# FrozenBurning/SceneDreamer

Measured on AMD Instinct MI355X. Metric: rendered frames/sec @960×540, 24 samples/ray, scene_size 2048; HBM GB/s, higher is better.
Workload: dtype f16 (3-term split MFMA, f32 accumulate; f32 hash grid); 1 GPU; 960x540, num_samples=24, scene_size=2048, cam pattern 0 (pose stride 2 of 40 poses), 1 frame per rank per step; apron=minimal, parallelism=frames x1

## Files before the change

scenedreamer_amd/cnn.py:

```python
import ctypes
import os

import torch

from . import capi

_LAYERS = {"conv1": (64, 1), "conv2a": (256, 9), "conv2b": (256, 9), "conv3a": (256, 9), "conv3b": (256, 9),
           "conv4a": (256, 1), "conv4b": (256, 1)}
_3X3 = ("conv2a", "conv2b", "conv3a", "conv3b")
CNN_LADDER = (1, "1113", "1133", 3)


def form_key(terms3x3):
    if isinstance(terms3x3, (tuple, list)):
        terms3x3 = "".join(str(int(t)) for t in terms3x3)
    if isinstance(terms3x3, str):
        terms3x3 = terms3x3.strip()
        if terms3x3 in ("1", "3"):
            return int(terms3x3)
        if not (len(terms3x3) == 4 and set(terms3x3) <= {"1", "3"}):
            raise ValueError(f"3x3 precision form {terms3x3!r}: expected 1, 3 or four characters of 1 / 3 (conv2a, conv2b, conv3a, conv3b), e.g. 1113")
        return 1 if terms3x3 == "1111" else 3 if terms3x3 == "3333" else terms3x3
    assert int(terms3x3) in (1, 3), terms3x3
    return int(terms3x3)


def form_terms(terms3x3):
    k = form_key(terms3x3)
    return (k,) * 4 if isinstance(k, int) else tuple(int(c) for c in k)


def form_cost(terms3x3):
    return sum(form_terms(terms3x3))


class MfmaCNN:
    def __init__(self, R, terms3x3, chain=None):
        self.R = R
        self.form = form_key(terms3x3)
        per3x3 = dict(zip(_3X3, form_terms(terms3x3)))
        if chain is None:
            chain = os.environ.get("SDN_CNN_CHAIN", "1") != "0"
        self.chain = bool(chain)
        self.terms = {n: per3x3.get(n, 3) for n in _LAYERS}
        lib = capi.lib()
        w = R.w
        self.packed = {}
        with torch.cuda.device(R.dev):
            for n, (cin, taps) in _LAYERS.items():
                wt = w[f"denoiser.{n}.weight"]
                assert tuple(wt.shape[:2]) == (256, cin) and wt.shape[2] * wt.shape[3] == taps, (n, tuple(wt.shape))
                buf = torch.empty(lib.sdn_conv_packed_weight_bytes(cin, taps, self.terms[n]), dtype=torch.uint8, device=R.dev)
                capi.check(lib.sdn_conv_pack_weights(wt.contiguous().data_ptr(), cin, taps, self.terms[n], buf.data_ptr(),
                                                     capi.current_stream(R.dev)), "sdn_conv_pack_weights")
                self.packed[n] = buf
        self.w4 = w["denoiser.conv4.weight"].reshape(3, 256).contiguous()
        self.b4 = w["denoiser.conv4.bias"].contiguous()
        self._planes = {}
        if self.chain:
            from . import fused
            try:
                fused.check_trunk_range(w["denoiser.conv4a.weight"], [w["denoiser.conv4b.weight"], w["denoiser.conv4.weight"]],
                                        lib.sdn_field_trunk_shift(), "render CNN tail")
            except fused.TrunkRangeError as e:
                import warnings
                warnings.warn(f"MfmaCNN: {e}; head and tail run as sdn_conv launches instead (no pre-tanh output)")
                self.chain = False
        if self.chain:
            with torch.cuda.device(R.dev):
                self.chain_packed = torch.empty(lib.sdn_conv_chain_packed_weight_bytes(), dtype=torch.uint8, device=R.dev)
                w4a = w["denoiser.conv4a.weight"].reshape(256, 256).contiguous()
                w4b = w["denoiser.conv4b.weight"].reshape(256, 256).contiguous()
                capi.check(lib.sdn_conv_chain_pack_weights(w4a.data_ptr(), w4b.data_ptr(), self.w4.data_ptr(),
                                                           self.chain_packed.data_ptr(), capi.current_stream(R.dev)),
                           "sdn_conv_chain_pack_weights")
                c = torch.zeros(lib.sdn_conv_chain_consts_floats(), device=R.dev)
                c[0:256] = w["denoiser.conv4a.bias"]
                c[256:512] = w["denoiser.conv4b.bias"]
                c[512:515] = self.b4
                self.chain_consts = c
                self.head_packed = torch.empty(lib.sdn_conv_head_packed_weight_bytes(), dtype=torch.uint8, device=R.dev)
                w1 = w["denoiser.conv1.weight"].reshape(256, 64).contiguous()
                capi.check(lib.sdn_conv_head_pack_weights(w1.data_ptr(), self.head_packed.data_ptr(), capi.current_stream(R.dev)),
                           "sdn_conv_head_pack_weights")
                self.head_bias = w["denoiser.conv1.bias"].contiguous()

    def _buffers(self, H, W):
        key = (H, W)
        if key not in self._planes:
            hb, wb = ctypes.c_int(), ctypes.c_int()
            capi.lib().sdn_conv_plane_dims(H, W, ctypes.byref(hb), ctypes.byref(wb))
            n = hb.value * wb.value * 256
            mk = lambda: torch.zeros(n, dtype=torch.float16, device=self.R.dev)
            while len(self._planes) >= 2:
                self._planes.pop(next(iter(self._planes)))
            self._planes[key] = dict(a=(mk(), mk()), b=(mk(), mk()))
        return self._planes[key]

    def _adapt(self):
        t = self.R.cnn_adapt
        if getattr(self, "_adapt_src", None) is not t:
            self._adapt_src = t
            self._adapt_vecs = [c[0].contiguous() for c in torch.chunk(t, 4, dim=-1)]
        return self._adapt_vecs

    def _conv(self, src, name, H, W, bias=None, resid=None, resid_planes=None, mod=None, dst=None, out32=None, proj=None,
              img=None):
        p = lambda t: t.data_ptr() if t is not None else None
        cin, taps = _LAYERS[name]
        with torch.cuda.device(self.R.dev):
            capi.check(capi.lib().sdn_conv(src[0].data_ptr(), src[1].data_ptr(), cin, taps, self.terms[name],
                                           self.packed[name].data_ptr(),
                                           p(bias), p(resid), resid_planes[0].data_ptr() if resid_planes else None,
                                           resid_planes[1].data_ptr() if resid_planes else None,
                                           p(mod[0]) if mod else None, p(mod[1]) if mod else None,
                                           dst[0].data_ptr() if dst else None,
                                           dst[1].data_ptr() if dst and dst[1] is not None else None, p(out32),
                                           p(proj[0]) if proj else None, p(proj[1]) if proj else None, p(img),
                                           H, W, 0, capi.current_stream(self.R.dev)), "sdn_conv")

    FLOP_PER_PIXEL = {"head (conv1)": 2 * 64 * 256, "conv2a": 2 * 9 * 256 * 256, "conv2b": 2 * 9 * 256 * 256, "conv3a": 2 * 9 * 256 * 256,
                      "conv3b": 2 * 9 * 256 * 256, "chain (conv4a, conv4b, conv4)": 2 * (2 * 256 * 256 + 256 * 3)}

    def __call__(self, net_out, raw=None, timers=None):
        last = [None]

        def tick(name=None):
            if timers is None:
                return
            e = torch.cuda.Event(enable_timing=True)
            e.record()
            if name is not None:
                timers.setdefault(name, []).append((last[0], e))
            last[0] = e
        if raw is not None and not self.chain:
            raise ValueError("the pre-tanh output is produced by the chained tail (chain=True)")
        R, w = self.R, self.R.w
        _, H, W, _ = net_out.shape
        buf = self._buffers(H, W)
        A, B = buf["a"], buf["b"]
        a = self._adapt()
        bias = lambda n: w.get(f"denoiser.{n}.bias")
        x = net_out.reshape(H * W, 64).contiguous()
        img = torch.empty(1, 3, H, W, device=R.dev)
        tick()
        if self.chain:
            with torch.cuda.device(R.dev):
                capi.check(capi.lib().sdn_conv_head(x.data_ptr(), self.head_packed.data_ptr(), self.head_bias.data_ptr(),
                                                    A[0].data_ptr(), A[1].data_ptr(), H, W, 0, capi.current_stream(R.dev)),
                           "sdn_conv_head")
        else:
            with torch.cuda.device(R.dev):
                capi.check(capi.lib().sdn_conv_planes_from_f32(x.data_ptr(), 64, B[0].data_ptr(), B[1].data_ptr(), H, W,
                                                               capi.current_stream(R.dev)), "sdn_conv_planes_from_f32")
            self._conv(B, "conv1", H, W, bias=bias("conv1"), dst=A)
        inner = lambda consumer: (B[0], None) if self.terms[consumer] == 1 else B
        tick("head (conv1)")
        self._conv(A, "conv2a", H, W, bias=bias("conv2a"), dst=inner("conv2b"))
        tick("conv2a")
        self._conv(B, "conv2b", H, W, bias=bias("conv2b"), resid_planes=A, mod=(a[0], a[1]), dst=A)
        tick("conv2b")
        self._conv(A, "conv3a", H, W, bias=bias("conv3a"), dst=inner("conv3b"))
        tick("conv3a")
        self._conv(B, "conv3b", H, W, bias=bias("conv3b"), resid_planes=A, mod=(a[2], a[3]), dst=A)
        tick("conv3b")
        if self.chain:
            with torch.cuda.device(R.dev):
                capi.check(capi.lib().sdn_conv_chain(A[0].data_ptr(), A[1].data_ptr(), self.chain_packed.data_ptr(),
                                                     self.chain_consts.data_ptr(), img.data_ptr(),
                                                     raw.data_ptr() if raw is not None else None, H, W, 0,
                                                     capi.current_stream(R.dev)), "sdn_conv_chain")
            tick("chain (conv4a, conv4b, conv4)")
            return img
        self._conv(A, "conv4a", H, W, bias=bias("conv4a"), dst=B)
        self._conv(B, "conv4b", H, W, bias=bias("conv4b"), resid_planes=A, proj=(self.w4, self.b4), img=img)
        return img


class F32CNN:

    FLOP_PER_PIXEL = {"conv1": 2 * 64 * 256, "conv2a": 2 * 9 * 256 * 256, "conv2b": 2 * 9 * 256 * 256, "conv3a": 2 * 9 * 256 * 256,
                      "conv3b": 2 * 9 * 256 * 256, "conv4a": 2 * 256 * 256, "conv4b (+ conv4)": 2 * (256 * 256 + 256 * 3)}

    def __init__(self, R):
        self.R = R
        self._planes = {}
        lib = capi.lib()
        w = R.w
        self.packed = {}
        with torch.cuda.device(R.dev):
            for n, (cin, taps) in _LAYERS.items():
                wt = w[f"denoiser.{n}.weight"]
                assert tuple(wt.shape[:2]) == (256, cin) and wt.shape[2] * wt.shape[3] == taps, (n, tuple(wt.shape))
                buf = torch.empty(lib.sdn_conv_f32_packed_weight_bytes(cin, taps), dtype=torch.uint8, device=R.dev)
                capi.check(lib.sdn_conv_pack_weights_f32(wt.contiguous().data_ptr(), cin, taps, buf.data_ptr(), capi.current_stream(R.dev)),
                           "sdn_conv_pack_weights_f32")
                self.packed[n] = buf
        self.bias = {n: (w[f"denoiser.{n}.bias"].contiguous() if f"denoiser.{n}.bias" in w else None) for n in _LAYERS}
        self.w4 = w["denoiser.conv4.weight"].reshape(3, 256).contiguous()
        self.b4 = w["denoiser.conv4.bias"].contiguous()

    def _buffers(self, H, W):
# ... 55 lines not shown
```

scenedreamer_amd/csrc/cnn.hip:

```cpp
#include <hip/hip_fp16.h>

#include <cstdlib>

#include "mfma_common.h"
#include "sdn_common.h"

namespace {

typedef _Float16 half4 __attribute__((ext_vector_type(4)));

constexpr int CH = 256;
constexpr int A_BYTES = 16384;
constexpr int B_BYTES = 2048;
constexpr int WAVES = 8;
constexpr int SLOT_BYTES = A_BYTES + WAVES * B_BYTES;
constexpr int NSLOT = 5;
constexpr int AHEAD = 4;
constexpr int DMA_PER_SLOT = 4;
constexpr int TILE_W = 8, TILE_H = 4;
constexpr int PATCH_W = 16, PATCH_H = 16;

struct ConvParams {
    const _Float16 *xh, *xl;
    const char *wpk;
    int ksteps;
    const float *bias;
    const float *resid;
    const _Float16 *rh, *rl;
    const float *mod_w;
    const float *mod_b;
    _Float16 *oh, *ol;
    float *of32;
    const float *proj_w;
    const float *proj_b;
    float *img;
    int H, W, Hb, Wb;
    long chunk_bytes;
    unsigned row_inc, chunk_inc;
    int gx, gy, n_groups;
};

struct Stream {
    unsigned long off;
    int tap;
    int w;
};

template <int TAPS>
__device__ __forceinline__ void stream_advance_k(const ConvParams &p, Stream &st) {
    if constexpr (TAPS == 9) {
        unsigned inc = ((0x24u >> st.tap) & 1u) ? p.row_inc : 32u;
        inc = st.tap == 8 ? p.chunk_inc : inc;
        st.off += inc;
        st.tap = st.tap == 8 ? 0 : st.tap + 1;
    } else {
        st.off += (unsigned long)p.chunk_bytes;
    }
}

struct SlotIssue {
    const char *w;
    const char *a0, *a1;
    unsigned voff;
    char *dst;
};

template <int TAPS, int TERMS>
__device__ __forceinline__ SlotIssue stream_next_slot(const ConvParams &p, Stream &st, char *lds, int pos, int wave, unsigned voff, int ksteps) {
    SlotIssue si;
    si.w = p.wpk + (size_t)st.w * A_BYTES + wave * 2048;
    si.a0 = (const char *)p.xh + st.off;
    if constexpr (TERMS == 1) {
        stream_advance_k<TAPS>(p, st);
        si.a1 = (const char *)p.xh + st.off;
    } else {
        si.a1 = (const char *)p.xl + st.off;
    }
    stream_advance_k<TAPS>(p, st);
    st.w++;
    if (st.w == ksteps) {
        st.w = 0;
        st.off = 0;
    }
    si.voff = voff;
    si.dst = lds + pos * SLOT_BYTES;
    return si;
}

template <int TAPS, int TERMS, int U>
__device__ __forceinline__ void stream_chunk(const ConvParams &p, Stream &st, SlotIssue &sn, char *lds, int &pos, int wave,
                                             unsigned voff_sel, int ksteps) {
    if constexpr (U == 0) {
        asm volatile("" : "+s"(st.w));
        sn.w = p.wpk + (size_t)st.w * A_BYTES + wave * 2048;
        sn.dst = lds + pos * SLOT_BYTES;
        pos = pos + 1 == NSLOT ? 0 : pos + 1;
        asm volatile("" ::"s"(sn.w), "s"(pos));
    } else if constexpr (U == 1) {
        asm volatile("" : "+s"(st.tap));
        sn.a0 = (const char *)p.xh + st.off;
        if constexpr (TERMS == 1) stream_advance_k<TAPS>(p, st);
        asm volatile("" ::"s"(sn.a0), "s"(st.off), "s"(st.tap));
    } else if constexpr (U == 2) {
        asm volatile("" : "+s"(st.tap));
        sn.a1 = (const char *)(TERMS == 1 ? p.xh : p.xl) + st.off;
        stream_advance_k<TAPS>(p, st);
        asm volatile("" ::"s"(sn.a1), "s"(st.off), "s"(st.tap));
    } else {
        asm volatile("" : "+s"(st.w));
        st.w++;
        if (st.w == ksteps) {
            st.w = 0;
            st.off = 0;
        }
        asm volatile("" ::"s"(st.w), "s"(st.off));
    }
}

template <int PIECE>
__device__ __forceinline__ void issue_piece(const SlotIssue &si, int wave, int lane) {
    if constexpr (PIECE == 0) __builtin_amdgcn_global_load_lds((glb_char *)(si.w + (unsigned)(lane * 16)), (lds_char *)(si.dst + wave * 2048), 16, 0, 0);
    if constexpr (PIECE == 1) __builtin_amdgcn_global_load_lds((glb_char *)(si.w + (unsigned)(lane * 16)), (lds_char *)(si.dst + wave * 2048), 16, 1024, 0);
    if constexpr (PIECE == 2) __builtin_amdgcn_global_load_lds((glb_char *)(si.a0 + si.voff), (lds_char *)(si.dst + A_BYTES + wave * B_BYTES), 16, 0, 0);
    if constexpr (PIECE == 3) __builtin_amdgcn_global_load_lds((glb_char *)(si.a1 + si.voff), (lds_char *)(si.dst + A_BYTES + wave * B_BYTES + 1024), 16, 0, 0);
}

template <int TAPS, int TERMS, int DBG, int U>
__device__ __forceinline__ void conv_unit(f32x16 (&acc)[8], half8 (&a)[4][4], half8 (&bcur)[2], half8 (&bnext)[2], unsigned slot,
                                          unsigned slot_n, unsigned b_off, const SlotIssue &si, int wave, int lane,
                                          const ConvParams &p, Stream &st, SlotIssue &sn, char *lds, int &pos_issue, unsigned voff_sel, int ksteps) {
    constexpr int ib = 2 * U;
    half8(&au)[4] = a[U];
    half8(&nx)[4] = a[(U + 2) & 3];
    const unsigned src = U < 2 ? slot : slot_n;
    constexpr int OFF = ((U + 2) & 3) * 4096;
    if constexpr (!(DBG & 64)) lds_wait<U == 3 ? 6 : 4>();
#define SDN_GAP(K) \
    if constexpr (K == 0 && !(DBG & 1)) issue_piece<U>(si, wave, lane); \
    if constexpr (K == 0 && U == 2 && !(DBG & 64)) { ds_read16<0>(bnext[0], slot_n + b_off); ds_read16<1024>(bnext[1], slot_n + b_off); } \
    if constexpr (K >= 1 && K <= 4 && !(DBG & 64)) ds_read16<OFF + (K - 1) * 1024>(nx[K - 1], src); \
    if constexpr (K == 2) stream_chunk<TAPS, TERMS, U>(p, st, sn, lds, pos_issue, wave, voff_sel, ksteps); \
    __builtin_amdgcn_sched_barrier(0);
    if constexpr (DBG & 16) {
        asm volatile("" ::"v"(au[0]), "v"(au[1]), "v"(au[2]), "v"(au[3]), "v"(bcur[0]), "v"(bcur[1]));
        SDN_GAP(0) SDN_GAP(1) SDN_GAP(2) SDN_GAP(3) SDN_GAP(4)
    } else if constexpr (TERMS == 1) {
        acc[ib] = mfma16(au[0], bcur[0], acc[ib]);
        __builtin_amdgcn_sched_barrier(0);
        SDN_GAP(0)
        acc[ib + 1] = mfma16(au[2], bcur[0], acc[ib + 1]);
        SDN_GAP(1) SDN_GAP(2)
        acc[ib] = mfma16(au[1], bcur[1], acc[ib]);
        SDN_GAP(3)
        acc[ib + 1] = mfma16(au[3], bcur[1], acc[ib + 1]);
        SDN_GAP(4)
    } else {
        acc[ib] = mfma16(au[0], bcur[0], acc[ib]);
        __builtin_amdgcn_sched_barrier(0);
        SDN_GAP(0)
        acc[ib + 1] = mfma16(au[2], bcur[0], acc[ib + 1]);
        SDN_GAP(1)
        acc[ib] = mfma16(au[1], bcur[0], acc[ib]);
        SDN_GAP(2)
        acc[ib + 1] = mfma16(au[3], bcur[0], acc[ib + 1]);
        SDN_GAP(3)
        acc[ib] = mfma16(au[0], bcur[1], acc[ib]);
        SDN_GAP(4)
        acc[ib + 1] = mfma16(au[2], bcur[1], acc[ib + 1]);
        __builtin_amdgcn_sched_barrier(0);
    }
#undef SDN_GAP
}

__device__ __forceinline__ long lane_pixel_offset(const ConvParams &p, int grp, int wave, int lane, int &py, int &px) {
    const int gyi = grp / p.gx, gxi = grp - gyi * p.gx;
    const int j = lane & 31, h = lane >> 5;
    py = gyi * PATCH_H + (wave >> 1) * TILE_H + (j >> 3);
    px = gxi * PATCH_W + (wave & 1) * TILE_W + (j & 7);
    return ((long)(py + 1) * p.Wb + (px + 1)) * 32 + h * 16;
}

template <int TAPS, int DBG, int TERMS, int EPI>
__global__ __launch_bounds__(512, 2) void conv_kernel(const ConvParams p) {
    __shared__ __attribute__((aligned(1024))) char lds[NSLOT * SLOT_BYTES];
    const int lane = threadIdx.x & 63;
    const int wave = __builtin_amdgcn_readfirstlane(threadIdx.x >> 6);
    const int h = lane >> 5;

    int grp = blockIdx.x;
    if (grp >= p.n_groups) return;
    const unsigned tap0 = TAPS == 9 ? (unsigned)(p.Wb + 1) * 32u : 0u;
    int py, px;
    unsigned voff = (unsigned)lane_pixel_offset(p, grp, wave, lane, py, px) - tap0;
    int grp_n = grp + gridDim.x;
    int pyn, pxn;
    unsigned voff_n = grp_n < p.n_groups ? (unsigned)lane_pixel_offset(p, grp_n, wave, lane, pyn, pxn) - tap0 : voff;

    const int ksteps = p.ksteps;
    {
        const int n_mine = (p.n_groups - (int)blockIdx.x + (int)gridDim.x - 1) / (int)gridDim.x;
        const int n_max = (p.n_groups + (int)gridDim.x - 1) / (int)gridDim.x;
        if (!(DBG & 2048) && n_mine < n_max) {
            const int phase = (blockIdx.x >> 3) & 15;
            const int naps = (phase * (ksteps * 1400 + 20000)) >> (4 + 13);
            for (int i = 0; i < naps; i++) __builtin_amdgcn_s_sleep(127);
        }
    }
    Stream st{0ul, 0, 0};
    int pos_issue = 0, pos_use = 0;
#pragma unroll
    for (int q = 0; q < AHEAD; q++) {
        const SlotIssue si = stream_next_slot<TAPS, TERMS>(p, st, lds, pos_issue, wave, voff, ksteps);
        issue_piece<0>(si, wave, lane);
        issue_piece<1>(si, wave, lane);
        issue_piece<2>(si, wave, lane);
        issue_piece<3>(si, wave, lane);
        pos_issue = pos_issue + 1 == NSLOT ? 0 : pos_issue + 1;
    }
    SlotIssue si = stream_next_slot<TAPS, TERMS>(p, st, lds, pos_issue, wave, AHEAD < ksteps ? voff : voff_n, ksteps);
    pos_issue = pos_issue + 1 == NSLOT ? 0 : pos_issue + 1;

    half8 a[4][4];
    half8 b[2][2];
    const unsigned lds_lane = lds_addr(lds) + lane * 16;
    const unsigned b_off = A_BYTES + wave * B_BYTES;
    bool first_patch = true;
    asm volatile("s_waitcnt vmcnt(%0)" ::"n"((AHEAD - 1) * DMA_PER_SLOT) : "memory");
    __builtin_amdgcn_s_barrier();
    ds_read16<0>(b[0][0], lds_lane + b_off);
    ds_read16<1024>(b[0][1], lds_lane + b_off);
    lds_unit<0>(lds_lane, a[0]);
    lds_unit<1>(lds_lane, a[1]);

    while (true) {
        f32x16 acc[8];
#pragma unroll
        for (int ib = 0; ib < 8; ib++)
#pragma unroll
            for (int r = 0; r < 16; r++) acc[ib][r] = 0.f;
#pragma unroll 1
        for (int kt2 = 0; kt2 < ksteps; kt2 += 2) {
#pragma unroll
            for (int par = 0; par < 2; par++) {
                const int kt = kt2 + par;
                SlotIssue sn;
                si.voff = kt + AHEAD < ksteps ? voff : voff_n;
                const unsigned voff_sel = si.voff;
                const unsigned slot = lds_lane + pos_use * SLOT_BYTES;
                pos_use = pos_use + 1 == NSLOT ? 0 : pos_use + 1;
                const unsigned slot_n = lds_lane + pos_use * SLOT_BYTES;
                asm volatile("" ::"v"(voff_sel), "v"(slot), "v"(slot_n));
                __builtin_amdgcn_sched_barrier(0);
                if (kt >= AHEAD - 1 || first_patch) asm volatile("s_waitcnt vmcnt(%0)" ::"n"((AHEAD - 2) * DMA_PER_SLOT) : "memory");
                if constexpr (!(DBG & 2)) __builtin_amdgcn_s_barrier();
                __builtin_amdgcn_sched_barrier(0);
                conv_unit<TAPS, TERMS, DBG, 0>(acc, a, b[par], b[par ^ 1], slot, slot_n, b_off, si, wave, lane, p, st, sn, lds, pos_issue, voff_sel, ksteps);
                conv_unit<TAPS, TERMS, DBG, 1>(acc, a, b[par], b[par ^ 1], slot, slot_n, b_off, si, wave, lane, p, st, sn, lds, pos_issue, voff_sel, ksteps);
                conv_unit<TAPS, TERMS, DBG, 2>(acc, a, b[par], b[par ^ 1], slot, slot_n, b_off, si, wave, lane, p, st, sn, lds, pos_issue, voff_sel, ksteps);
                conv_unit<TAPS, TERMS, DBG, 3>(acc, a, b[par], b[par ^ 1], slot, slot_n, b_off, si, wave, lane, p, st, sn, lds, pos_issue, voff_sel, ksteps);
                si = sn;
            }
        }
        asm volatile("s_waitcnt vmcnt(0) lgkmcnt(0)" ::: "memory");
        first_patch = false;

        const bool in_frame = py < p.H && px < p.W;
        if (in_frame) {
            const long orow = (long)py * p.W + px;
            const long ppix = (long)(py + 1) * p.Wb + (px + 1);
            float pj[3] = {0.f, 0.f, 0.f};
            const long plane_px = (long)p.Hb * p.Wb;
            constexpr bool SPEC = EPI != 255;
            const bool has_bias = SPEC ? !(EPI & 8) : p.bias != nullptr, has_rp = SPEC ? bool(EPI & 1) : p.rh != nullptr;
            const bool has_mod = SPEC ? bool(EPI & 2) : p.mod_w != nullptr, has_r32 = !SPEC && p.resid;
            const bool has_proj = !SPEC && p.proj_w, has_o32 = !SPEC && p.of32;
            const bool has_oh = SPEC || p.oh, has_ol = SPEC ? bool(EPI & 16) : p.ol != nullptr;
            int he = h;
            asm volatile("" : "+v"(he));
#pragma unroll
            for (int ib = 0; ib < 8; ib++) {
#pragma unroll
                for (int q = 0; q < 2; q++) {
                    const int c0 = 32 * ib + 16 * he + 8 * q;
                    const long po = ((long)(2 * ib + he) * plane_px + ppix) * 16 + 8 * q;
                    float v[8];
#pragma unroll
                    for (int e = 0; e < 8; e++) v[e] = acc[ib][8 * q + e];
                    if (has_bias) {
                        const float4 b0 = *reinterpret_cast<const float4 *>(p.bias + c0), b1 = *reinterpret_cast<const float4 *>(p.bias + c0 + 4);
                        v[0] += b0.x; v[1] += b0.y; v[2] += b0.z; v[3] += b0.w; v[4] += b1.x; v[5] += b1.y; v[6] += b1.z; v[7] += b1.w;
                    }
                    if (has_r32) {
                        const float4 r0 = *reinterpret_cast<const float4 *>(p.resid + orow * CH + c0);
                        const float4 r1 = *reinterpret_cast<const float4 *>(p.resid + orow * CH + c0 + 4);
                        v[0] = r0.x + v[0]; v[1] = r0.y + v[1]; v[2] = r0.z + v[2]; v[3] = r0.w + v[3];
                        v[4] = r1.x + v[4]; v[5] = r1.y + v[5]; v[6] = r1.z + v[6]; v[7] = r1.w + v[7];
                    } else if (has_rp) {
                        const half8 h8 = *reinterpret_cast<const half8 *>(p.rh + po);
                        const half8 l8 = *reinterpret_cast<const half8 *>(p.rl + po);
#pragma unroll
                        for (int e = 0; e < 8; e++) v[e] = ((float)h8[e] + (float)l8[e]) + v[e];
                    }
                    if (has_mod) {
#pragma unroll
                        for (int e4 = 0; e4 < 2; e4++) {
                            const float4 mw = *reinterpret_cast<const float4 *>(p.mod_w + c0 + 4 * e4);
                            const float4 mb = *reinterpret_cast<const float4 *>(p.mod_b + c0 + 4 * e4);
                            v[4 * e4] = v[4 * e4] * (mw.x + 1.f) + mb.x; v[4 * e4 + 1] = v[4 * e4 + 1] * (mw.y + 1.f) + mb.y;
                            v[4 * e4 + 2] = v[4 * e4 + 2] * (mw.z + 1.f) + mb.z; v[4 * e4 + 3] = v[4 * e4 + 3] * (mw.w + 1.f) + mb.w;
                        }
                    }
#pragma unroll
                    for (int e = 0; e < 8; e++) v[e] = vmax(v[e], 0.2f * v[e]);
                    if (has_proj) {
#pragma unroll
                        for (int c = 0; c < 3; c++) {
                            const float4 w0 = *reinterpret_cast<const float4 *>(p.proj_w + c * CH + c0);
                            const float4 w1 = *reinterpret_cast<const float4 *>(p.proj_w + c * CH + c0 + 4);
                            pj[c] += w0.x * v[0] + w0.y * v[1] + w0.z * v[2] + w0.w * v[3] + w1.x * v[4] + w1.y * v[5] + w1.z * v[6] + w1.w * v[7];
                        }
                    }
#pragma unroll
                    for (int e = 0; e < 8; e++) acc[ib][8 * q + e] = v[e];
                }
            }
            if (has_o32 || has_oh) {
#pragma unroll
                for (int ib = 0; ib < 8; ib++) {
#pragma unroll
                    for (int q = 0; q < 2; q++) {
                        const int c0 = 32 * ib + 16 * he + 8 * q;
                        const long po = ((long)(2 * ib + he) * plane_px + ppix) * 16 + 8 * q;
                        float v[8];
#pragma unroll
                        for (int e = 0; e < 8; e++) v[e] = acc[ib][8 * q + e];
                        if (has_o32) {
                            *reinterpret_cast<float4 *>(p.of32 + orow * CH + c0) = make_float4(v[0], v[1], v[2], v[3]);
                            *reinterpret_cast<float4 *>(p.of32 + orow * CH + c0 + 4) = make_float4(v[4], v[5], v[6], v[7]);
                        }
                        if (has_oh) {
                            half8 hv, lv;
#pragma unroll
                            for (int e = 0; e < 8; e += 2) {
                                const half2v hp = cvt_rtn(v[e], v[e + 1]);
                                hv[e] = hp[0]; hv[e + 1] = hp[1];
                                const half2v lp = cvt_rtn(v[e] - (float)hp[0], v[e + 1] - (float)hp[1]);
                                lv[e] = lp[0]; lv[e + 1] = lp[1];
                            }
                            *reinterpret_cast<half8 *>(p.oh + po) = hv;
                            if (has_ol) *reinterpret_cast<half8 *>(p.ol + po) = lv;
                        }
                    }
                }
            }
            if (has_proj) {
#pragma unroll
                for (int c = 0; c < 3; c++) {
                    const float t = pj[c] + __shfl_xor(pj[c], 32);
                    if (h == 0) p.img[(long)c * p.H * p.W + orow] = tanhf(t + p.proj_b[c]);
                }
            }
        }
        grp = grp_n;
        if (grp >= p.n_groups) break;
        voff = voff_n;
        py = pyn;
        px = pxn;
        grp_n = grp + gridDim.x;
        voff_n = grp_n < p.n_groups ? (unsigned)lane_pixel_offset(p, grp_n, wave, lane, pyn, pxn) - tap0 : voff;
    }
    asm volatile("s_waitcnt vmcnt(0)" ::: "memory");
    __builtin_amdgcn_s_barrier();
}

__global__ __launch_bounds__(256) void pack_conv_kernel(const float *__restrict__ W, half8 *__restrict__ out, int cin, int taps, int terms) {
    const size_t g = (size_t)blockIdx.x * 256 + threadIdx.x;
    const int nslots = (cin / 16) * taps / (terms == 1 ? 2 : 1);
    if (g >= (size_t)nslots * 8 * 64) return;
    const int lane = (int)(g % 64);
    const int ib = (int)((g / 64) % 8);
    const int t = (int)(g / (64 * 8));
    const int i32 = lane & 31, h = lane >> 5;
    const int co = 32 * ib + 16 * ((i32 >> 2) & 1) + 4 * (i32 >> 3) + (i32 & 3);
    half8 hi, lo;
    if (terms == 1) {
#pragma unroll
        for (int kk = 0; kk < 2; kk++) {
            const int k = 2 * t + kk, s = k / taps, tap = k - taps * s;
#pragma unroll
            for (int e = 0; e < 8; e++) {
                const _Float16 vh = (_Float16)W[((size_t)co * cin + 16 * s + 8 * h + e) * taps + tap];
                if (kk == 0) hi[e] = vh;
                else lo[e] = vh;
            }
        }
    } else {
        const int s = t / taps, tap = t - taps * s;
#pragma unroll
        for (int e = 0; e < 8; e++) {
            const int ci = 16 * s + 8 * h + e;
            const float v = W[((size_t)co * cin + ci) * taps + tap];
            const _Float16 vh = (_Float16)v;
            hi[e] = vh;
            lo[e] = (_Float16)(v - (float)vh);
        }
    }
    const size_t base = ((size_t)t * 16 + (size_t)(ib / 2) * 4 + (ib & 1) * 2) * 64 + lane;
    out[base] = hi;
    out[base + 64] = lo;
}

__global__ __launch_bounds__(256) void planes_kernel(const float *__restrict__ x, _Float16 *__restrict__ oh,
                                                     _Float16 *__restrict__ ol, int H, int W, int Hb, int Wb, int C) {
    const long n = (long)H * W * (C / 4);
    for (long i = (long)blockIdx.x * 256 + threadIdx.x; i < n; i += (long)gridDim.x * 256) {
        const long pix = i / (C / 4);
        const int c0 = (int)(i % (C / 4)) * 4;
        const int y = (int)(pix / W), xx = (int)(pix % W);
        const float4 v = *reinterpret_cast<const float4 *>(x + pix * C + c0);
        const half2v h0 = cvt_rtn(v.x, v.y), h1 = cvt_rtn(v.z, v.w);
        const half2v l0 = cvt_rtn(v.x - (float)h0[0], v.y - (float)h0[1]);
        const half2v l1 = cvt_rtn(v.z - (float)h1[0], v.w - (float)h1[1]);
        half4 hv, lv;
        hv[0] = h0[0]; hv[1] = h0[1]; hv[2] = h1[0]; hv[3] = h1[1];
        lv[0] = l0[0]; lv[1] = l0[1]; lv[2] = l1[0]; lv[3] = l1[1];
        const long o = ((long)(c0 >> 4) * ((long)Hb * Wb) + (long)(y + 1) * Wb + (xx + 1)) * 16 + (c0 & 15);
        *reinterpret_cast<half4 *>(oh + o) = hv;
        *reinterpret_cast<half4 *>(ol + o) = lv;
    }
}

}

extern "C" {

void sdn_conv_plane_dims(int H, int W, int *Hb, int *Wb) {
    *Hb = sdn::div_up(H, PATCH_H) * PATCH_H + 2;
    *Wb = sdn::div_up(W, PATCH_W) * PATCH_W + 2;
}

static bool conv_shape_ok(int cin, int taps, int terms) {
    if (terms != 1 && terms != 3) return false;
    if (terms == 1 && !(taps == 9 && cin == 256)) return false;
    return (taps == 9 && cin == 256) || (taps == 1 && cin >= 64 && cin <= 256 && cin % 16 == 0);
}
#define SDN_CONV_SHAPES "supported: 3x3 256->256 (terms 1 or 3) and 1x1 (64..256, multiple of 16)->256 (terms 3)"

static int conv_slots(int cin, int taps, int terms) { return (cin / 16) * taps / (terms == 1 ? 2 : 1); }

size_t sdn_conv_packed_weight_bytes(int cin, int taps, int terms) {
    return conv_shape_ok(cin, taps, terms) ? (size_t)conv_slots(cin, taps, terms) * A_BYTES : 0;
}

int sdn_conv_pack_weights(const float *w_oihw, int cin, int taps, int terms, void *packed, sdn_stream_t stream) {
    SDN_REQUIRE(w_oihw && packed, "sdn_conv_pack_weights: null pointer");
    SDN_REQUIRE(conv_shape_ok(cin, taps, terms), "sdn_conv_pack_weights: " SDN_CONV_SHAPES);
    const size_t n = (size_t)conv_slots(cin, taps, terms) * 8 * 64;
    hipLaunchKernelGGL(pack_conv_kernel, dim3((unsigned)sdn::div_up<size_t>(n, 256)), dim3(256), 0, (hipStream_t)stream,
                       w_oihw, (half8 *)packed, cin, taps, terms);
    return sdn::check_launch("sdn_conv_pack_weights");
}

int sdn_conv_planes_from_f32(const float *x, int channels, void *out_hi, void *out_lo, int H, int W, sdn_stream_t stream) {
    SDN_REQUIRE(x && out_hi && out_lo && H > 0 && W > 0, "sdn_conv_planes_from_f32: bad argument");
    SDN_REQUIRE(channels >= 16 && channels <= 256 && channels % 16 == 0, "sdn_conv_planes_from_f32: channels must be a multiple of 16 in [16, 256]");
    int Hb, Wb;
    sdn_conv_plane_dims(H, W, &Hb, &Wb);
    hipLaunchKernelGGL(planes_kernel, dim3(2048), dim3(256), 0, (hipStream_t)stream, x, (_Float16 *)out_hi, (_Float16 *)out_lo,
                       H, W, Hb, Wb, channels);
    return sdn::check_launch("sdn_conv_planes_from_f32");
}

int sdn_conv(const void *in_hi, const void *in_lo, int cin, int taps, int terms, const void *packed, const float *bias, const float *resid,
             const void *resid_hi, const void *resid_lo, const float *mod_w, const float *mod_b, void *out_hi, void *out_lo,
             float *out_f32, const float *proj_w, const float *proj_b, float *out_img, int H, int W, int n_workgroups,
             sdn_stream_t stream) {
    SDN_REQUIRE(in_hi && packed && H > 0 && W > 0, "sdn_conv: bad argument");
    SDN_REQUIRE(conv_shape_ok(cin, taps, terms), "sdn_conv: " SDN_CONV_SHAPES);
    SDN_REQUIRE(in_lo || terms == 1, "sdn_conv: the 3-term product needs the lo input plane");
    SDN_REQUIRE(out_hi || out_f32 || out_img, "sdn_conv: no output requested");
    SDN_REQUIRE(out_hi || !out_lo, "sdn_conv: out_lo without out_hi");
    SDN_REQUIRE((mod_w == nullptr) == (mod_b == nullptr), "sdn_conv: mod_w and mod_b go together");
    SDN_REQUIRE((resid_hi == nullptr) == (resid_lo == nullptr) && !(resid && resid_hi), "sdn_conv: one residual form at most");
    SDN_REQUIRE(!(resid_hi && (resid_hi == in_hi || resid_lo == in_lo)), "sdn_conv: the residual planes must not be the input planes");
    SDN_REQUIRE((proj_w == nullptr) == (out_img == nullptr) && (proj_w == nullptr) == (proj_b == nullptr),
                "sdn_conv: proj_w, proj_b and out_img go together");
    ConvParams p;
    p.xh = (const _Float16 *)in_hi; p.xl = (const _Float16 *)in_lo; p.wpk = (const char *)packed;
    p.ksteps = conv_slots(cin, taps, terms);
    p.bias = bias; p.resid = resid; p.rh = (const _Float16 *)resid_hi; p.rl = (const _Float16 *)resid_lo; p.mod_w = mod_w; p.mod_b = mod_b;
    p.oh = (_Float16 *)out_hi; p.ol = (_Float16 *)out_lo; p.of32 = out_f32;
    p.proj_w = proj_w; p.proj_b = proj_b; p.img = out_img;
    p.H = H; p.W = W;
    sdn_conv_plane_dims(H, W, &p.Hb, &p.Wb);
    p.chunk_bytes = (long)p.Hb * p.Wb * 32;
    SDN_REQUIRE(p.chunk_bytes < (1l << 32), "sdn_conv: frame too large (a channel chunk of a plane must stay below 4 GiB)");
    p.row_inc = (unsigned)(p.Wb - 2) * 32u;
    p.chunk_inc = (unsigned)(p.chunk_bytes - 2l * (p.Wb + 1) * 32);
    p.gx = sdn::div_up(W, PATCH_W);
    p.gy = sdn::div_up(H, PATCH_H);
    p.n_groups = p.gx * p.gy;
    int wg = n_workgroups > 0 ? n_workgroups : 256;
    if (wg > p.n_groups) wg = p.n_groups;
    const bool rp = resid_hi != nullptr, md = mod_w != nullptr, pj = proj_w != nullptr, lo = out_lo != nullptr;
    int epi = 255;
    if (!resid && !out_f32 && !pj && out_hi) {
        if (bias && !rp && !md) epi = lo ? 16 : 0;
        else if (!bias && rp && md && lo) epi = 1 | 2 | 8 | 16;
    }
    int dbg = 0;
#ifdef SDN_MLP_ABLATION
    if (const char *e1 = getenv("SDN_CONV_DBG")) dbg = atoi(e1);
#endif
    const dim3 grid(wg), block(64 * WAVES);
    hipStream_t hs = (hipStream_t)stream;
#define SDN_LAUNCH(TAPS, DBG, TERMS, EPI) hipLaunchKernelGGL((conv_kernel<TAPS, DBG, TERMS, EPI>), grid, block, 0, hs, p)
    if (taps == 1) {
        if (epi == 16) SDN_LAUNCH(1, 0, 3, 16);
        else SDN_LAUNCH(1, 0, 3, 255);
    } else if (terms == 1) {
        if (dbg && (epi == 0 || epi == 16)) {
#ifdef SDN_MLP_ABLATION
            switch (dbg) {
                case 1: SDN_LAUNCH(9, 1, 1, 16); break;
                case 2: SDN_LAUNCH(9, 2, 1, 16); break;
                case 3: SDN_LAUNCH(9, 3, 1, 16); break;
                case 16: SDN_LAUNCH(9, 16, 1, 16); break;
                case 17: SDN_LAUNCH(9, 17, 1, 16); break;
                case 19: SDN_LAUNCH(9, 19, 1, 16); break;
                case 64: SDN_LAUNCH(9, 64, 1, 16); break;
                case 65: SDN_LAUNCH(9, 65, 1, 16); break;
                case 67: SDN_LAUNCH(9, 67, 1, 16); break;
                default: SDN_LAUNCH(9, 0, 1, 16); break;
            }
#endif
        } else if (epi == 0) SDN_LAUNCH(9, 0, 1, 0);
        else if (epi == 16) SDN_LAUNCH(9, 0, 1, 16);
        else if (epi == 27) SDN_LAUNCH(9, 0, 1, 27);
        else SDN_LAUNCH(9, 0, 1, 255);
    } else {
        if (epi == 16) SDN_LAUNCH(9, 0, 3, 16);
        else if (epi == 27) SDN_LAUNCH(9, 0, 3, 27);
        else SDN_LAUNCH(9, 0, 3, 255);
    }
#undef SDN_LAUNCH
    return sdn::check_launch("sdn_conv");
}

}
```

Baseline: 55.42 frames/s.

## Balance 3x3 conv tail work with edge strips and output-channel split of leftover patches

For the specialized 3x3 conv epilogues, edge patches are re-tiled into wide bottom or tall right strips so partial 16x16 patches waste fewer lanes. The leftover patches that do not fill a whole wave of workgroups are split by output-channel quarters or halves across otherwise idle workgroups, each loading only its part of the weights. The epilogue also prefetches bias, residual and modulation loads ahead of use. This aims to reduce the final-wave tail imbalance and edge waste, at the cost of extra template instantiations, code size and more complex index math.

```diff
diff --git a/scenedreamer_amd/cnn.py b/scenedreamer_amd/cnn.py
--- a/scenedreamer_amd/cnn.py
+++ b/scenedreamer_amd/cnn.py
@@ -42,6 +42,7 @@
         if chain is None:
             chain = os.environ.get("SDN_CNN_CHAIN", "1") != "0"
         self.chain = bool(chain)
+        self.n_workgroups = 0
         self.terms = {n: per3x3.get(n, 3) for n in _LAYERS}
         lib = capi.lib()
         w = R.w
@@ -117,7 +118,7 @@
                                            dst[0].data_ptr() if dst else None,
                                            dst[1].data_ptr() if dst and dst[1] is not None else None, p(out32),
                                            p(proj[0]) if proj else None, p(proj[1]) if proj else None, p(img),
-                                           H, W, 0, capi.current_stream(self.R.dev)), "sdn_conv")
+                                           H, W, self.n_workgroups, capi.current_stream(self.R.dev)), "sdn_conv")
 
     FLOP_PER_PIXEL = {"head (conv1)": 2 * 64 * 256, "conv2a": 2 * 9 * 256 * 256, "conv2b": 2 * 9 * 256 * 256, "conv3a": 2 * 9 * 256 * 256,
                       "conv3b": 2 * 9 * 256 * 256, "chain (conv4a, conv4b, conv4)": 2 * (2 * 256 * 256 + 256 * 3)}
diff --git a/scenedreamer_amd/csrc/cnn.hip b/scenedreamer_amd/csrc/cnn.hip
--- a/scenedreamer_amd/csrc/cnn.hip
+++ b/scenedreamer_amd/csrc/cnn.hip
@@ -16,7 +16,6 @@
 constexpr int SLOT_BYTES = A_BYTES + WAVES * B_BYTES;
 constexpr int NSLOT = 5;
 constexpr int AHEAD = 4;
-constexpr int DMA_PER_SLOT = 4;
 constexpr int TILE_W = 8, TILE_H = 4;
 constexpr int PATCH_W = 16, PATCH_H = 16;
 
@@ -38,7 +37,25 @@
     long chunk_bytes;
     unsigned row_inc, chunk_inc;
     int gx, gy, n_groups;
+    int split;
+    int strips;
+    int gxf, gyf, n_int;
+    int n_bot, bot_w;
+    int n_right, right_h;
 };
+
+template <int NU> constexpr int dma_per_slot() { return NU == 4 ? 4 : 3; }
+template <int NU> constexpr int wave_weight_bytes() { return NU == 4 ? 2048 : 1024; }
+template <int NU> constexpr int gap_piece(int U, int K) {
+    if (NU == 4) return K == 0 ? U : -1;
+    if (NU == 2) return K == 0 ? (U == 0 ? 0 : 2) : (U == 1 && K == 2) ? 3 : -1;
+    return K == 0 ? 0 : K == 1 ? 2 : K == 3 ? 3 : -1;
+}
+template <int NU> constexpr int gap_chunk(int U, int K) {
+    if (NU == 4) return K == 2 ? U : -1;
+    if (NU == 2) return K == 2 ? 2 * U : K == 4 ? 2 * U + 1 : -1;
+    return K >= 1 ? K - 1 : -1;
+}
 
 struct Stream {
     unsigned long off;
@@ -66,9 +83,9 @@
 };
 
 template <int TAPS, int TERMS>
-__device__ __forceinline__ SlotIssue stream_next_slot(const ConvParams &p, Stream &st, char *lds, int pos, int wave, unsigned voff, int ksteps) {
+__device__ __forceinline__ SlotIssue stream_next_slot(const ConvParams &p, Stream &st, char *lds, int pos, int wofs, unsigned voff, int ksteps) {
     SlotIssue si;
-    si.w = p.wpk + (size_t)st.w * A_BYTES + wave * 2048;
+    si.w = p.wpk + (size_t)st.w * A_BYTES + wofs;
     si.a0 = (const char *)p.xh + st.off;
     if constexpr (TERMS == 1) {
         stream_advance_k<TAPS>(p, st);
@@ -88,11 +105,11 @@
 }
 
 template <int TAPS, int TERMS, int U>
-__device__ __forceinline__ void stream_chunk(const ConvParams &p, Stream &st, SlotIssue &sn, char *lds, int &pos, int wave,
+__device__ __forceinline__ void stream_chunk(const ConvParams &p, Stream &st, SlotIssue &sn, char *lds, int &pos, int wofs,
                                              unsigned voff_sel, int ksteps) {
     if constexpr (U == 0) {
         asm volatile("" : "+s"(st.w));
-        sn.w = p.wpk + (size_t)st.w * A_BYTES + wave * 2048;
+        sn.w = p.wpk + (size_t)st.w * A_BYTES + wofs;
         sn.dst = lds + pos * SLOT_BYTES;
         pos = pos + 1 == NSLOT ? 0 : pos + 1;
         asm volatile("" ::"s"(sn.w), "s"(pos));
@@ -117,29 +134,34 @@
     }
 }
 
-template <int PIECE>
+template <int PIECE, int NU = 4>
 __device__ __forceinline__ void issue_piece(const SlotIssue &si, int wave, int lane) {
-    if constexpr (PIECE == 0) __builtin_amdgcn_global_load_lds((glb_char *)(si.w + (unsigned)(lane * 16)), (lds_char *)(si.dst + wave * 2048), 16, 0, 0);
-    if constexpr (PIECE == 1) __builtin_amdgcn_global_load_lds((glb_char *)(si.w + (unsigned)(lane * 16)), (lds_char *)(si.dst + wave * 2048), 16, 1024, 0);
+    constexpr int WB = wave_weight_bytes<NU>();
+    static_assert(PIECE != 1 || NU == 4, "a part's weights are one piece per wave");
+    if constexpr (PIECE == 0) __builtin_amdgcn_global_load_lds((glb_char *)(si.w + (unsigned)(lane * 16)), (lds_char *)(si.dst + wave * WB), 16, 0, 0);
+    if constexpr (PIECE == 1) __builtin_amdgcn_global_load_lds((glb_char *)(si.w + (unsigned)(lane * 16)), (lds_char *)(si.dst + wave * WB), 16, 1024, 0);
     if constexpr (PIECE == 2) __builtin_amdgcn_global_load_lds((glb_char *)(si.a0 + si.voff), (lds_char *)(si.dst + A_BYTES + wave * B_BYTES), 16, 0, 0);
     if constexpr (PIECE == 3) __builtin_amdgcn_global_load_lds((glb_char *)(si.a1 + si.voff), (lds_char *)(si.dst + A_BYTES + wave * B_BYTES + 1024), 16, 0, 0);
 }
 
-template <int TAPS, int TERMS, int DBG, int U>
-__device__ __forceinline__ void conv_unit(f32x16 (&acc)[8], half8 (&a)[4][4], half8 (&bcur)[2], half8 (&bnext)[2], unsigned slot,
+template <int TAPS, int TERMS, int DBG, int NU, int PAR, int U>
+__device__ __forceinline__ void conv_unit(f32x16 (&acc)[2 * NU], half8 (&a)[4][4], half8 (&bcur)[2], half8 (&bnext)[2], unsigned slot,
                                           unsigned slot_n, unsigned b_off, const SlotIssue &si, int wave, int lane,
-                                          const ConvParams &p, Stream &st, SlotIssue &sn, char *lds, int &pos_issue, unsigned voff_sel, int ksteps) {
+                                          const ConvParams &p, Stream &st, SlotIssue &sn, char *lds, int &pos_issue, unsigned voff_sel, int ksteps,
+                                          int wofs) {
     constexpr int ib = 2 * U;
-    half8(&au)[4] = a[U];
-    half8(&nx)[4] = a[(U + 2) & 3];
-    const unsigned src = U < 2 ? slot : slot_n;
-    constexpr int OFF = ((U + 2) & 3) * 4096;
-    if constexpr (!(DBG & 64)) lds_wait<U == 3 ? 6 : 4>();
+    constexpr int CUR = NU == 4 ? U : NU == 2 ? 2 * PAR + U : PAR;
+    half8(&au)[4] = a[CUR];
+    half8(&nx)[4] = a[NU == 1 ? (PAR ^ 1) : ((CUR + 2) & 3)];
+    const unsigned src = (NU == 4 && U < 2) ? slot : slot_n;
+    constexpr int OFF = NU == 4 ? ((U + 2) & 3) * 4096 : U * 4096;
+    constexpr int UB = NU == 4 ? 2 : 0;
+    if constexpr (!(DBG & 64)) lds_wait<NU == 1 ? 0 : (U == ((UB + 1) & 3) ? 6 : 4)>();
 #define SDN_GAP(K) \
-    if constexpr (K == 0 && !(DBG & 1)) issue_piece<U>(si, wave, lane); \
-    if constexpr (K == 0 && U == 2 && !(DBG & 64)) { ds_read16<0>(bnext[0], slot_n + b_off); ds_read16<1024>(bnext[1], slot_n + b_off); } \
+    if constexpr (!(DBG & 1)) issue_piece<gap_piece<NU>(U, K), NU>(si, wave, lane); \
+    if constexpr (K == 0 && U == UB && !(DBG & 64)) { ds_read16<0>(bnext[0], slot_n + b_off); ds_read16<1024>(bnext[1], slot_n + b_off); } \
     if constexpr (K >= 1 && K <= 4 && !(DBG & 64)) ds_read16<OFF + (K - 1) * 1024>(nx[K - 1], src); \
-    if constexpr (K == 2) stream_chunk<TAPS, TERMS, U>(p, st, sn, lds, pos_issue, wave, voff_sel, ksteps); \
+    if constexpr (gap_chunk<NU>(U, K) >= 0) stream_chunk<TAPS, TERMS, gap_chunk<NU>(U, K)>(p, st, sn, lds, pos_issue, wofs, voff_sel, ksteps); \
     __builtin_amdgcn_sched_barrier(0);
     if constexpr (DBG & 16) {
         asm volatile("" ::"v"(au[0]), "v"(au[1]), "v"(au[2]), "v"(au[3]), "v"(bcur[0]), "v"(bcur[1]));
@@ -173,69 +195,105 @@
 }
 
 __device__ __forceinline__ long lane_pixel_offset(const ConvParams &p, int grp, int wave, int lane, int &py, int &px) {
-    const int gyi = grp / p.gx, gxi = grp - gyi * p.gx;
     const int j = lane & 31, h = lane >> 5;
-    py = gyi * PATCH_H + (wave >> 1) * TILE_H + (j >> 3);
-    px = gxi * PATCH_W + (wave & 1) * TILE_W + (j & 7);
-    return ((long)(py + 1) * p.Wb + (px + 1)) * 32 + h * 16;
-}
-
-template <int TAPS, int DBG, int TERMS, int EPI>
-__global__ __launch_bounds__(512, 2) void conv_kernel(const ConvParams p) {
-    __shared__ __attribute__((aligned(1024))) char lds[NSLOT * SLOT_BYTES];
-    const int lane = threadIdx.x & 63;
-    const int wave = __builtin_amdgcn_readfirstlane(threadIdx.x >> 6);
+    if (!p.strips) {
+        const int gyi = grp / p.gx, gxi = grp - gyi * p.gx;
+        py = gyi * PATCH_H + (wave >> 1) * TILE_H + (j >> 3);
+        px = gxi * PATCH_W + (wave & 1) * TILE_W + (j & 7);
+        return ((long)(py + 1) * p.Wb + (px + 1)) * 32 + h * 16;
+    }
+    int x0 = p.gxf * PATCH_W, y0 = p.gyf * PATCH_H, tx = wave & 1, ty = wave >> 1;
+    int xlim = 0x7fffffff, ylim = 0x7fffffff;
+    if (grp < p.n_int) {
+        const int gyi = grp / p.gxf, gxi = grp - gyi * p.gxf;
+        x0 = gxi * PATCH_W;
+        y0 = gyi * PATCH_H;
+    } else if (grp < p.n_int + p.n_bot) {
+        x0 = (grp - p.n_int) * p.bot_w;
+        xlim = p.gxf * PATCH_W;
+        if (p.bot_w == 64) { tx = wave; ty = 0; }
+        else if (p.bot_w == 32) { tx = wave & 3; ty = wave >> 2; }
+    } else if (grp < p.n_int + p.n_bot + p.n_right) {
+        y0 = (grp - p.n_int - p.n_bot) * p.right_h;
+        ylim = p.gyf * PATCH_H;
+        if (p.right_h == 32) { tx = 0; ty = wave; }
+    }
+    py = y0 + ty * TILE_H + (j >> 3);
+    px = x0 + tx * TILE_W + (j & 7);
+    const int ly = py < ylim ? py : ylim - 1, lx = px < xlim ? px : xlim - 1;
+    if (py >= ylim || px >= xlim) py = p.H;
+    return ((long)(ly + 1) * p.Wb + (lx + 1)) * 32 + h * 16;
+}
+
+struct EpiLoads {
+    float4 b0, b1;
+    half8 h8, l8;
+    float4 mw[2], mb[2];
+};
+template <int EPI>
+__device__ __forceinline__ void epi_issue(const ConvParams &p, int c0, long po, EpiLoads &L) {
+    if constexpr (!(EPI & 8)) {
+        L.b0 = *reinterpret_cast<const float4 *>(p.bias + c0);
+        L.b1 = *reinterpret_cast<const float4 *>(p.bias + c0 + 4);
+    }
+    if constexpr (EPI & 1) {
+        L.h8 = *reinterpret_cast<const half8 *>(p.rh + po);
+        L.l8 = *reinterpret_cast<const half8 *>(p.rl + po);
+    }
+    if constexpr (EPI & 2) {
+#pragma unroll
+        for (int e4 = 0; e4 < 2; e4++) {
+            L.mw[e4] = *reinterpret_cast<const float4 *>(p.mod_w + c0 + 4 * e4);
+            L.mb[e4] = *reinterpret_cast<const float4 *>(p.mod_b + c0 + 4 * e4);
+        }
+    }
+}
+
+template <int TAPS, int DBG, int TERMS, int EPI, int NU>
+__device__ __forceinline__ void conv_patches(const ConvParams &p, char *lds, const int lane, const int wave, int grp, const int grp_end,
+                                             const int stride, const int part) {
+    constexpr int DPS = dma_per_slot<NU>();
     const int h = lane >> 5;
-
-    int grp = blockIdx.x;
-    if (grp >= p.n_groups) return;
     const unsigned tap0 = TAPS == 9 ? (unsigned)(p.Wb + 1) * 32u : 0u;
     int py, px;
     unsigned voff = (unsigned)lane_pixel_offset(p, grp, wave, lane, py, px) - tap0;
-    int grp_n = grp + gridDim.x;
+    int grp_n = grp + stride;
     int pyn, pxn;
-    unsigned voff_n = grp_n < p.n_groups ? (unsigned)lane_pixel_offset(p, grp_n, wave, lane, pyn, pxn) - tap0 : voff;
+    unsigned voff_n = grp_n < grp_end ? (unsigned)lane_pixel_offset(p, grp_n, wave, lane, pyn, pxn) - tap0 : voff;
 
     const int ksteps = p.ksteps;
-    {
-        const int n_mine = (p.n_groups - (int)blockIdx.x + (int)gridDim.x - 1) / (int)gridDim.x;
-        const int n_max = (p.n_groups + (int)gridDim.x - 1) / (int)gridDim.x;
-        if (!(DBG & 2048) && n_mine < n_max) {
-            const int phase = (blockIdx.x >> 3) & 15;
-            const int naps = (phase * (ksteps * 1400 + 20000)) >> (4 + 13);
-            for (int i = 0; i < naps; i++) __builtin_amdgcn_s_sleep(127);
-        }
-    }
+    const int wofs = (NU == 4 ? 0 : (NU == 2 ? part : part >> 1) * (A_BYTES / 2)) + wave * wave_weight_bytes<NU>();
+    const int ib0 = NU == 4 ? 0 : part * 2 * NU;
     Stream st{0ul, 0, 0};
     int pos_issue = 0, pos_use = 0;
 #pragma unroll
     for (int q = 0; q < AHEAD; q++) {
-        const SlotIssue si = stream_next_slot<TAPS, TERMS>(p, st, lds, pos_issue, wave, voff, ksteps);
-        issue_piece<0>(si, wave, lane);
-        issue_piece<1>(si, wave, lane);
-        issue_piece<2>(si, wave, lane);
-        issue_piece<3>(si, wave, lane);
+        const SlotIssue si = stream_next_slot<TAPS, TERMS>(p, st, lds, pos_issue, wofs, voff, ksteps);
+        issue_piece<0, NU>(si, wave, lane);
+        if constexpr (NU == 4) issue_piece<1, NU>(si, wave, lane);
+        issue_piece<2, NU>(si, wave, lane);
+        issue_piece<3, NU>(si, wave, lane);
         pos_issue = pos_issue + 1 == NSLOT ? 0 : pos_issue + 1;
     }
-    SlotIssue si = stream_next_slot<TAPS, TERMS>(p, st, lds, pos_issue, wave, AHEAD < ksteps ? voff : voff_n, ksteps);
+    SlotIssue si = stream_next_slot<TAPS, TERMS>(p, st, lds, pos_issue, wofs, AHEAD < ksteps ? voff : voff_n, ksteps);
     pos_issue = pos_issue + 1 == NSLOT ? 0 : pos_issue + 1;
 
     half8 a[4][4];
     half8 b[2][2];
-    const unsigned lds_lane = lds_addr(lds) + lane * 16;
-    const unsigned b_off = A_BYTES + wave * B_BYTES;
+    const unsigned lds_lane = lds_addr(lds) + lane * 16 + (NU == 1 ? (part & 1) * 4096 : 0);
+    const unsigned b_off = A_BYTES + wave * B_BYTES - (NU == 1 ? (part & 1) * 4096 : 0);
     bool first_patch = true;
-    asm volatile("s_waitcnt vmcnt(%0)" ::"n"((AHEAD - 1) * DMA_PER_SLOT) : "memory");
+    asm volatile("s_waitcnt vmcnt(%0)" ::"n"((AHEAD - 1) * DPS) : "memory");
     __builtin_amdgcn_s_barrier();
     ds_read16<0>(b[0][0], lds_lane + b_off);
     ds_read16<1024>(b[0][1], lds_lane + b_off);
     lds_unit<0>(lds_lane, a[0]);
-    lds_unit<1>(lds_lane, a[1]);
+    if constexpr (NU > 1) lds_unit<1>(lds_lane, a[1]);
 
     while (true) {
-        f32x16 acc[8];
-#pragma unroll
-        for (int ib = 0; ib < 8; ib++)
+        f32x16 acc[2 * NU];
+#pragma unroll
+        for (int ib = 0; ib < 2 * NU; ib++)
 #pragma unroll
             for (int r = 0; r < 16; r++) acc[ib][r] = 0.f;
 #pragma unroll 1
@@ -251,13 +309,14 @@
                 const unsigned slot_n = lds_lane + pos_use * SLOT_BYTES;
                 asm volatile("" ::"v"(voff_sel), "v"(slot), "v"(slot_n));
                 __builtin_amdgcn_sched_barrier(0);
-                if (kt >= AHEAD - 1 || first_patch) asm volatile("s_waitcnt vmcnt(%0)" ::"n"((AHEAD - 2) * DMA_PER_SLOT) : "memory");
+                if (kt >= AHEAD - 1 || first_patch) asm volatile("s_waitcnt vmcnt(%0)" ::"n"((AHEAD - 2) * DPS) : "memory");
                 if constexpr (!(DBG & 2)) __builtin_amdgcn_s_barrier();
                 __builtin_amdgcn_sched_barrier(0);
-                conv_unit<TAPS, TERMS, DBG, 0>(acc, a, b[par], b[par ^ 1], slot, slot_n, b_off, si, wave, lane, p, st, sn, lds, pos_issue, voff_sel, ksteps);
-                conv_unit<TAPS, TERMS, DBG, 1>(acc, a, b[par], b[par ^ 1], slot, slot_n, b_off, si, wave, lane, p, st, sn, lds, pos_issue, voff_sel, ksteps);
-                conv_unit<TAPS, TERMS, DBG, 2>(acc, a, b[par], b[par ^ 1], slot, slot_n, b_off, si, wave, lane, p, st, sn, lds, pos_issue, voff_sel, ksteps);
-                conv_unit<TAPS, TERMS, DBG, 3>(acc, a, b[par], b[par ^ 1], slot, slot_n, b_off, si, wave, lane, p, st, sn, lds, pos_issue, voff_sel, ksteps);
+#define SDN_UNIT(PAR, U) conv_unit<TAPS, TERMS, DBG, NU, PAR, U>(acc, a, b[PAR], b[PAR ^ 1], slot, slot_n, b_off, si, wave, lane, p, st, sn, lds, pos_issue, voff_sel, ksteps, wofs)
+#define SDN_UNITS(PAR) { SDN_UNIT(PAR, 0); if constexpr (NU > 1) SDN_UNIT(PAR, 1); if constexpr (NU > 2) { SDN_UNIT(PAR, 2); SDN_UNIT(PAR, 3); } }
+                if (par == 0) SDN_UNITS(0) else SDN_UNITS(1)
+#undef SDN_UNITS
+#undef SDN_UNIT
                 si = sn;
             }
         }
@@ -277,12 +336,51 @@
             const bool has_oh = SPEC || p.oh, has_ol = SPEC ? bool(EPI & 16) : p.ol != nullptr;
             int he = h;
             asm volatile("" : "+v"(he));
-#pragma unroll
-            for (int ib = 0; ib < 8; ib++) {
+            if constexpr (SPEC) {
+                constexpr int NIT = 4 * NU, AH = (EPI & 1) ? 1 : 2;
+                EpiLoads L[NIT];
+#pragma unroll
+                for (int it = 0; it < NIT; it++) {
+#pragma unroll
+                    for (int nx = (it == 0 ? 0 : it + AH); nx <= it + AH && nx < NIT; nx++) {
+                        const int ibn = ib0 + (nx >> 1), qn = nx & 1;
+                        epi_issue<EPI>(p, 32 * ibn + 16 * he + 8 * qn, ((long)(2 * ibn + he) * plane_px + ppix) * 16 + 8 * qn, L[nx]);
+                    }
+                    __builtin_amdgcn_sched_barrier(0);
+                    const int ib = it >> 1, q = it & 1;
+                    float v[8];
+#pragma unroll
+                    for (int e = 0; e < 8; e++) v[e] = acc[ib][8 * q + e];
+                    if constexpr (!(EPI & 8)) {
+                        const float4 b0 = L[it].b0, b1 = L[it].b1;
+                        v[0] += b0.x; v[1] += b0.y; v[2] += b0.z; v[3] += b0.w; v[4] += b1.x; v[5] += b1.y; v[6] += b1.z; v[7] += b1.w;
+                    }
+                    if constexpr (EPI & 1) {
+                        const half8 h8 = L[it].h8, l8 = L[it].l8;
+#pragma unroll
+                        for (int e = 0; e < 8; e++) v[e] = ((float)h8[e] + (float)l8[e]) + v[e];
+                    }
+                    if constexpr (EPI & 2) {
+#pragma unroll
+                        for (int e4 = 0; e4 < 2; e4++) {
+                            const float4 mw = L[it].mw[e4], mb = L[it].mb[e4];
+                            v[4 * e4] = v[4 * e4] * (mw.x + 1.f) + mb.x; v[4 * e4 + 1] = v[4 * e4 + 1] * (mw.y + 1.f) + mb.y;
+                            v[4 * e4 + 2] = v[4 * e4 + 2] * (mw.z + 1.f) + mb.z; v[4 * e4 + 3] = v[4 * e4 + 3] * (mw.w + 1.f) + mb.w;
+                        }
+                    }
+#pragma unroll
+                    for (int e = 0; e < 8; e++) v[e] = vmax(v[e], 0.2f * v[e]);
+#pragma unroll
+                    for (int e = 0; e < 8; e++) acc[ib][8 * q + e] = v[e];
+                    __builtin_amdgcn_sched_barrier(0);
+                }
+            }
+#pragma unroll
+            for (int ib = 0; ib < (SPEC ? 0 : 2 * NU); ib++) {
 #pragma unroll
                 for (int q = 0; q < 2; q++) {
-                    const int c0 = 32 * ib + 16 * he + 8 * q;
-                    const long po = ((long)(2 * ib + he) * plane_px + ppix) * 16 + 8 * q;
+                    const int c0 = 32 * (ib0 + ib) + 16 * he + 8 * q;
+                    const long po = ((long)(2 * (ib0 + ib) + he) * plane_px + ppix) * 16 + 8 * q;
                     float v[8];
 #pragma unroll
                     for (int e = 0; e < 8; e++) v[e] = acc[ib][8 * q + e];
@@ -325,12 +423,14 @@
                 }
             }
             if (has_o32 || has_oh) {
-#pragma unroll
-                for (int ib = 0; ib < 8; ib++) {
+                int hs = h;
+                asm volatile("" : "+v"(hs));
+#pragma unroll
+                for (int ib = 0; ib < 2 * NU; ib++) {
 #pragma unroll
                     for (int q = 0; q < 2; q++) {
-                        const int c0 = 32 * ib + 16 * he + 8 * q;
-                        const long po = ((long)(2 * ib + he) * plane_px + ppix) * 16 + 8 * q;
+                        const int c0 = 32 * (ib0 + ib) + 16 * hs + 8 * q;
+                        const long po = ((long)(2 * (ib0 + ib) + hs) * plane_px + ppix) * 16 + 8 * q;
                         float v[8];
 #pragma unroll
                         for (int e = 0; e < 8; e++) v[e] = acc[ib][8 * q + e];
@@ -362,15 +462,47 @@
             }
         }
         grp = grp_n;
-        if (grp >= p.n_groups) break;
+        if (grp >= grp_end) break;
         voff = voff_n;
         py = pyn;
         px = pxn;
-        grp_n = grp + gridDim.x;
-        voff_n = grp_n < p.n_groups ? (unsigned)lane_pixel_offset(p, grp_n, wave, lane, pyn, pxn) - tap0 : voff;
+        grp_n = grp + stride;
+        voff_n = grp_n < grp_end ? (unsigned)lane_pixel_offset(p, grp_n, wave, lane, pyn, pxn) - tap0 : voff;
     }
     asm volatile("s_waitcnt vmcnt(0)" ::: "memory");
     __builtin_amdgcn_s_barrier();
+}
+
+template <int TAPS, int DBG, int TERMS, int EPI>
+__global__ __launch_bounds__(512, 2) void conv_kernel(const ConvParams p) {
+    __shared__ __attribute__((aligned(1024))) char lds[NSLOT * SLOT_BYTES];
+    const int lane = threadIdx.x & 63;
+    const int wave = __builtin_amdgcn_readfirstlane(threadIdx.x >> 6);
+    const int blk = blockIdx.x, grid = gridDim.x;
+    if (blk >= p.n_groups) return;
+    constexpr bool SPLIT = TAPS == 9 && EPI != 255;
+    const int n_whole = SPLIT && p.split > 1 ? p.n_groups / grid * grid : p.n_groups;
+    const int r = p.n_groups - n_whole, n_parts = r * p.split;
+    {
+        const int n_mine = (p.n_groups - blk + grid - 1) / grid;
+        const int n_max = (p.n_groups + grid - 1) / grid;
+        const bool spared = r > 0 ? blk >= n_parts : n_mine < n_max;
+        if (!(DBG & 2048) && spared) {
+            const int phase = (blk >> 3) & 15;
+            const int naps = ((phase * (p.ksteps * 1400 + 20000)) >> (4 + 13)) / (r > 0 ? p.split : 1);
+            for (int i = 0; i < naps; i++) __builtin_amdgcn_s_sleep(127);
+        }
+    }
+    conv_patches<TAPS, DBG, TERMS, EPI, 4>(p, lds, lane, wave, blk, n_whole, grid, 0);
+    if constexpr (SPLIT) {
+        int lane2 = lane, wave2 = wave, blk2 = blk;
+        asm volatile("" : "+v"(lane2), "+s"(wave2), "+s"(blk2));
+        if (blk2 < n_parts) {
+            const int part = blk2 / r, grp = n_whole + (blk2 - part * r);
+            if (p.split == 2) conv_patches<TAPS, DBG, TERMS, EPI, 2>(p, lds, lane2, wave2, grp, grp + 1, 1, part);
+            else conv_patches<TAPS, DBG, TERMS, EPI, 1>(p, lds, lane2, wave2, grp, grp + 1, 1, part);
+        }
+    }
 }
 
 __global__ __launch_bounds__(256) void pack_conv_kernel(const float *__restrict__ W, half8 *__restrict__ out, int cin, int taps, int terms) {
@@ -508,6 +640,29 @@
         if (bias && !rp && !md) epi = lo ? 16 : 0;
         else if (!bias && rp && md && lo) epi = 1 | 2 | 8 | 16;
     }
+    int tail = 3;
+    if (const char *e0 = getenv("SDN_CONV_TAIL")) tail = atoi(e0);
+    p.split = 1;
+    p.strips = 0;
+    p.gxf = p.gyf = p.n_int = p.n_bot = p.n_right = 0;
+    p.bot_w = p.right_h = 16;
+    if (taps == 9 && epi != 255 && (tail & 2)) {
+        const int R = H % PATCH_H, C = W % PATCH_W;
+        p.strips = 1;
+        p.gxf = W / PATCH_W;
+        p.gyf = H / PATCH_H;
+        p.n_int = p.gxf * p.gyf;
+        p.bot_w = R <= 4 ? 64 : R <= 8 ? 32 : 16;
+        p.right_h = C <= 8 ? 32 : 16;
+        p.n_bot = R ? sdn::div_up(p.gxf * PATCH_W, p.bot_w) : 0;
+        p.n_right = C ? sdn::div_up(p.gyf * PATCH_H, p.right_h) : 0;
+        p.n_groups = p.n_int + p.n_bot + p.n_right + (R && C ? 1 : 0);
+        if (wg > p.n_groups) wg = p.n_groups;
+    }
+    if (taps == 9 && epi != 255 && (tail & 1)) {
+        const int r = p.n_groups % wg;
+        if (r > 0) p.split = 4 * r <= wg ? 4 : 2 * r <= wg ? 2 : 1;
+    }
     int dbg = 0;
 #ifdef SDN_MLP_ABLATION
     if (const char *e1 = getenv("SDN_CONV_DBG")) dbg = atoi(e1);
```

Result: no change. 55.34 frames/s (median of 3 runs) (-0.2%).
